# marcinmiklitz/pywindow

Measured on AMD Instinct MI355X. Metric: trajectory frames/sec full_analysis (pore+windows), CC3 1k-frame, higher is better.
Workload: dtype f64

## Files before the change

pywindow_amd/csrc/pw_kernels.hip:

```cpp
#include <hip/hip_runtime.h>
#include <atomic>
#include <stdio.h>
#include <stdlib.h>
#include <string.h>
#include <time.h>

#include <algorithm>
#include <mutex>
#include <new>

#include "../../include/pywindow_amd.h"
#include "pw_host.hpp"
#include <vector>
#include "pw_unit.hpp"
#include "pw_launch.hpp"

using namespace pw;

extern "C" int pw_hostpath_run(const pw_batch_in* in, unsigned stages, pw_unit_out* out, const pw_params* prm, int p_cap,
                               int threads, pw_unit_debug* dbg, pw_extra_window* xw, unsigned xw_cap, unsigned* xw_count);
extern "C" int pw_hostpath_default_threads(void);
extern "C" void pw_hostpath_math(int which, const double* x, const double* y, long n, double* out);
extern "C" size_t pw_internal_big_block_bytes(int nmax, int p_cap);
extern "C" int pw_internal_big_launch(void* stream, int grid, long n_units, const long* atom_offset, const double* xyz,
                                      const double* vdw, const double* mass, unsigned stages, int nmax, const PwWsArgs* wsa,
                                      unsigned char* blocks, size_t block_bytes, unsigned long long* counter, pw_unit_out* out,
                                      const pw_params* prm, const unsigned* rsq_tab, int vstride);

namespace {

thread_local char g_err[512] = "";
void set_err(const char* what, hipError_t e) {
    snprintf(g_err, sizeof(g_err), "%s: %s", what, hipGetErrorString(e));
}
#define HIP_TRY(call)                         \
    do {                                      \
        hipError_t e_ = (call);               \
        if (e_ != hipSuccess) {               \
            set_err(#call, e_);               \
            return PW_E_HIP;                  \
        }                                     \
    } while (0)

#define PW_ON_DEVICE(dev)                     \
    DeviceScope dev_scope_;                   \
    HIP_TRY(dev_scope_.enter(dev))

constexpr int PW_SETS = 4;

constexpr size_t PW_KERNEL_STATIC_LDS = 1024;

constexpr unsigned MASK_ANY = 0xffffffffu;
constexpr unsigned MASK_CHAINS = PW_STAGE_BASIC | PW_STAGE_OPT | PW_STAGE_MERGE;
constexpr unsigned MASK_WINDOWS = PW_STAGE_WINDOWS | PW_STAGE_REUSE_OPT | PW_STAGE_MERGE | PW_STAGE_COM_ONLY;
constexpr unsigned MASK_WINDOWS_AVG = MASK_WINDOWS | PW_STAGE_AVG;

__global__ void __launch_bounds__(256) pw_nb_build_kernel(unsigned* __restrict__ off, unsigned short* __restrict__ idx,
                                                          double* __restrict__ bound, double* __restrict__ unit) {
    __shared__ double ux[PW_NB_PMAX], uy[PW_NB_PMAX], uz[PW_NB_PMAX];
    const int P = PW_NB_PMAX - (int)blockIdx.x;
    Sphere sp;
    sp.init(1.0, P);
    for (int k = threadIdx.x; k < P; k += blockDim.x) sp.point(k, &ux[k], &uy[k], &uz[k]);
    __syncthreads();
    const unsigned first = nb_dense_offset(P);
    if (threadIdx.x == 0) off[P] = first;
    if (unit)
        for (int k = threadIdx.x; k < P; k += blockDim.x) {
            double* q = unit + 3 * ((size_t)first + k);
            q[0] = ux[k]; q[1] = uy[k]; q[2] = uz[k];
        }
    for (int k = threadIdx.x; k < P; k += blockDim.x)
        nb_build_point(P, k, ux, uy, uz, idx + (size_t)(first + k) * PW_NB_K, bound + first + k);
}

__device__ inline bool wait_for_unit(const unsigned long long* ready, long u, int* error_flag, long long limit) {
    if (!ready) return true;
    long long t0 = wall_clock64();
    unsigned long long seen = ~0ull;
    for (;;) {
        const unsigned long long have = __hip_atomic_load(ready, __ATOMIC_RELAXED, __HIP_MEMORY_SCOPE_SYSTEM);
        if ((long)have > u && !(have >> 63)) break;
        __builtin_amdgcn_s_sleep(16);
        if (have != seen) { seen = have; t0 = wall_clock64(); }
        if ((have >> 63) || wall_clock64() - t0 > limit) {
            if (error_flag) atomicExch(error_flag, (have >> 63) ? 3 : 2);
            return false;
        }
    }
    __builtin_amdgcn_fence(__ATOMIC_ACQUIRE, "");
    asm volatile("s_waitcnt vmcnt(0)" ::: "memory");
    return true;
}
template <int NW, unsigned MASK>
__global__ void __launch_bounds__(NW * 64, 2)
pw_analyse_kernel(long n_units, const long* __restrict__ atom_offset, const double* __restrict__ xyz,
                  const double* __restrict__ vdw, const double* __restrict__ mass, unsigned stages,
                  int nmax, int nrot, int nlb, int nframes, int lean, PwWsArgs wsa, unsigned long long* counter,
                  pw_unit_out* __restrict__ out, int role, UnitQueue* queue, int* __restrict__ slots,
                  pw_params prm_in, const unsigned* __restrict__ rsq_tab, int vstride,
                  const unsigned long long* __restrict__ ready, const unsigned char* __restrict__ tmpl) {
    extern __shared__ __attribute__((aligned(16))) unsigned char lds[];
    __shared__ long s_unit;
    __shared__ UnitShared s_sh;
    __shared__ pw_params s_prm;
    static_assert(sizeof(UnitShared) + sizeof(pw_params) + 16 <= PW_KERNEL_STATIC_LDS, "static LDS of the analysis kernels");
    using T = DeviceTeam<NW>;
    if (role == PW_ROLE_PRODUCER) {
        __builtin_amdgcn_s_setprio(3);
        if (threadIdx.x == 0) atomicAdd(&queue->started, 1);
    }
    TeamWorkspace* ws = (TeamWorkspace*)wsa.ws + blockIdx.x;
#ifdef PW_PROFILE
    if (threadIdx.x < 32) pw_prof_lds[threadIdx.x] = 0;
#ifdef PW_BARRIER_PROF
    if (threadIdx.x < 8) pw_bar_acc[threadIdx.x] = 0;
#endif
#endif
    if (threadIdx.x == 0) {
        s_sh.carve(lds, nmax, nrot, nlb, nframes, lean, wsa.p_cap);
        s_prm = prm_in;
        bind_workspace(ws, wsa, blockIdx.x, rsq_tab, team_slab_bytes(wsa.p_cap), team_adj_words(wsa.p_cap));
    }
    __syncthreads();
    constexpr bool STATE_IN_LDS = MASK == MASK_CHAINS;
    UnitShared sh_stack;
    if (!STATE_IN_LDS) sh_stack.carve(lds, nmax, nrot, nlb, nframes, lean, wsa.p_cap);
    UnitShared& sh = STATE_IN_LDS ? (UnitShared&)s_sh : sh_stack;
    const pw_params& prm = STATE_IN_LDS ? (const pw_params&)s_prm : prm_in;
    for (;;) {
        if (role == PW_ROLE_CONSUMER) {
            if (threadIdx.x == 0) {
                long pos = (long)atomicAdd(&queue->head, 1ull);
                long u = -1;
                if (pos < n_units) {
                    long long t0 = wall_clock64();
#ifdef PW_PROFILE
                    const long long t_begin = t0;
#endif
                    unsigned long long seen = ~0ull;
                    int spins = 0;
                    for (;;) {
                        int v = __hip_atomic_load(&slots[pos], __ATOMIC_RELAXED, __HIP_MEMORY_SCOPE_AGENT);
                        if (v >= 0) {
                            u = v;
#ifdef PW_PROFILE
                            atomicAdd(&pw_prof_lds[1], (unsigned long long)(wall_clock64() - t_begin));
#endif
                            break;
                        }
                        __builtin_amdgcn_s_sleep(32);
                        if (__hip_atomic_load(&queue->error, __ATOMIC_RELAXED, __HIP_MEMORY_SCOPE_AGENT) != 0) break;
                        if ((++spins & 15) == 0) {
                            const unsigned long long pub = __hip_atomic_load(&queue->tail, __ATOMIC_RELAXED, __HIP_MEMORY_SCOPE_AGENT);
                            if (pub != seen) { seen = pub; t0 = wall_clock64(); }
                        }
                        if (wall_clock64() - t0 > wsa.wait_ticks) {
                            atomicExch(&queue->error, 1);
                            break;
                        }
                    }
                    __builtin_amdgcn_fence(__ATOMIC_ACQUIRE, "agent");
                    asm volatile("s_waitcnt vmcnt(0)" ::: "memory");
                }
                s_unit = u;
            }
        } else {
            if (threadIdx.x == 0) {
                long u = (long)atomicAdd(counter, 1ull);
                if (u < n_units && !wait_for_unit(ready, u, &queue->error, wsa.stream_wait_ticks)) u = n_units;
                s_unit = u < n_units ? u : -1;
            }
        }
        __syncthreads();
        long u = s_unit;
        __syncthreads();
        if (u < 0) break;
        long a0 = atom_offset[u];
        int n = (int)(atom_offset[u + 1] - a0);
        const long v0 = a0 * vstride;
        if (threadIdx.x == 0) ws->unit = u;
        analyse_unit<T>(sh, ws, n, xyz + 3 * a0, vdw + v0, mass + v0, stages & MASK, out + u, prm, vstride == 0 ? tmpl : nullptr);
        if (role == PW_ROLE_PRODUCER) {
            if (threadIdx.x == 0) {
                asm volatile("s_waitcnt vmcnt(0)" ::: "memory");
                __builtin_amdgcn_fence(__ATOMIC_RELEASE, "agent");
                asm volatile("s_waitcnt vmcnt(0)" ::: "memory");
                long pos = (long)atomicAdd(&queue->tail, 1ull);
                __hip_atomic_store(&slots[pos], (int)u, __ATOMIC_RELAXED, __HIP_MEMORY_SCOPE_AGENT);
            }
        }
    }
#ifdef PW_PROFILE
    __syncthreads();
    if (threadIdx.x < 32 && pw_prof_lds[threadIdx.x]) atomicAdd(&ws->prof[threadIdx.x], pw_prof_lds[threadIdx.x]);
#endif
}

__global__ void pw_gate_kernel(UnitQueue* queue, int expected, unsigned long long* timeouts, long long limit) {
    if (threadIdx.x != 0) return;
    long long t0 = wall_clock64();
    int seen = -1;
    for (;;) {
        const int started = __hip_atomic_load(&queue->started, __ATOMIC_RELAXED, __HIP_MEMORY_SCOPE_AGENT);
        if (started >= expected) break;
        __builtin_amdgcn_s_sleep(16);
        if (started != seen) { seen = started; t0 = wall_clock64(); }
        if (wall_clock64() - t0 > limit) {
            atomicAdd(timeouts, 1ull << 32);
            if (started == 0) atomicCAS(&queue->error, 0, 4);
            break;
        }
    }
}

__global__ void pw_tail_gate_kernel(const UnitQueue* prev, unsigned long long need, unsigned long long* timeouts) {
    if (threadIdx.x != 0) return;
    long long t0 = wall_clock64();
    while (__hip_atomic_load(&prev->tail, __ATOMIC_RELAXED, __HIP_MEMORY_SCOPE_AGENT) < need) {
        __builtin_amdgcn_s_sleep(32);
        if (wall_clock64() - t0 > 2000000ll) { atomicAdd(timeouts, 1ull); break; }
    }
}

__global__ void pw_head_gate_kernel(const UnitQueue* prev, unsigned long long need, unsigned long long* timeouts) {
    if (threadIdx.x != 0) return;
    long long t0 = wall_clock64();
    while (__hip_atomic_load(&prev->head, __ATOMIC_RELAXED, __HIP_MEMORY_SCOPE_AGENT) < need) {
        __builtin_amdgcn_s_sleep(32);
        if (wall_clock64() - t0 > 2000000ll) { atomicAdd(timeouts, 1ull << 16); break; }
    }
}

__global__ void pw_probe_kernel(int* started, int expected, int* together) {
    if (threadIdx.x != 0) return;
    atomicAdd(started, 1);
    long long t0 = wall_clock64();
    while (__hip_atomic_load(started, __ATOMIC_RELAXED, __HIP_MEMORY_SCOPE_AGENT) < expected) {
        __builtin_amdgcn_s_sleep(16);
        if (wall_clock64() - t0 > 1000000ll) return;
    }
    atomicAdd(together, 1);
}

template <int NW>
__global__ void __launch_bounds__(NW * 64) pw_dbscan_kernel(const double* __restrict__ pts, int n, double eps,
                                                            int lds_bytes, TeamWorkspace* ws, int p_cap,
                                                            unsigned long long* adj_base, const int* __restrict__ ident,
                                                            int* __restrict__ labels, int* __restrict__ n_clusters) {
    using T = DeviceTeam<NW>;
    extern __shared__ __attribute__((aligned(16))) unsigned char lds[];
    __shared__ unsigned long long bits[3][PW_DBSCAN_MAX / 64];
    if (threadIdx.x == 0) { ws->adj = adj_base; ws->p_cap = p_cap; }
    __syncthreads();
    ScratchArena arena;
    arena.cur = (unsigned char*)lds;
    arena.left = (size_t)lds_bytes;
    int* lab = (int*)arena.take((size_t)n * 4);
    if (!lab) lab = labels;
    auto PT = [n](int k, int c) { return c * n + k; };
    int k = team_dbscan<T>((PW_LDS unsigned long long*)bits[0], (PW_LDS unsigned long long*)bits[1],
                           (PW_LDS unsigned long long*)bits[2], arena, ws, pts, PT, ident, n, eps, lab);
    if (lab != labels)
        for (int i = threadIdx.x; i < n; i += NW * 64) labels[i] = lab[i];
    if (threadIdx.x == 0) *n_clusters = k;
}

template <int NW>
__global__ void __launch_bounds__(NW * 64) pw_pairwise_sum_kernel(const double* __restrict__ a, long n,
                                                                   double* __restrict__ scratch, int use_global,
                                                                   double* __restrict__ out) {
    using T = DeviceTeam<NW>;
    __shared__ int s_tab[324];
    __shared__ double s_acc[8 * 160];
    __shared__ double s_leaf[256];
    __shared__ double s_slot;
    int* tab = use_global ? (int*)(scratch + 8 * 160 + 256) : (int*)s_tab;
    double* acc = use_global ? scratch : (double*)s_acc;
// ... 1724 lines not shown
        if (d_p) (void)hipFree(d_p);
        if (d_i) (void)hipFree(d_i);
        if (d_l) (void)hipFree(d_l);
        if (d_ws) (void)hipFree(d_ws);
        if (d_adj) (void)hipFree(d_adj);
    };
#define DB_TRY(call)                                   \
    do {                                               \
        hipError_t e_ = (call);                        \
        if (e_ != hipSuccess) {                        \
            set_err(#call, e_);                        \
            cleanup();                                 \
            return PW_E_HIP;                           \
        }                                              \
    } while (0)
    std::vector<double> soa((size_t)3 * n);
    std::vector<int> ident((size_t)n);
    for (int64_t i = 0; i < n; ++i) {
        for (int k = 0; k < 3; ++k) soa[(size_t)k * n + i] = points[3 * i + k];
        ident[i] = (int)i;
    }
    DB_TRY(hipMalloc((void**)&d_p, sizeof(double) * 3 * n));
    DB_TRY(hipMalloc((void**)&d_i, sizeof(int) * n));
    DB_TRY(hipMalloc((void**)&d_l, sizeof(int) * (n + 1)));
    DB_TRY(hipMalloc((void**)&d_ws, sizeof(TeamWorkspace)));
    const int p_cap = round_p_cap((long)n);
    DB_TRY(hipMalloc((void**)&d_adj, sizeof(unsigned long long) * team_adj_words(p_cap)));
    DB_TRY(hipMemcpyAsync(d_p, soa.data(), sizeof(double) * 3 * n, hipMemcpyHostToDevice, c->stream));
    DB_TRY(hipMemcpyAsync(d_i, ident.data(), sizeof(int) * n, hipMemcpyHostToDevice, c->stream));
    const int lds_bytes = (mode & 2) ? 0 : 96 * 1024;
    if (mode & 1) {
        DB_TRY(hipFuncSetAttribute((const void*)pw_dbscan_kernel<1>, hipFuncAttributeMaxDynamicSharedMemorySize, 96 * 1024));
        hipLaunchKernelGGL(pw_dbscan_kernel<1>, dim3(1), dim3(64), lds_bytes, c->stream, d_p, (int)n, eps, lds_bytes, d_ws, p_cap,
                           d_adj, d_i, d_l, d_l + n);
    } else {
        DB_TRY(hipFuncSetAttribute((const void*)pw_dbscan_kernel<4>, hipFuncAttributeMaxDynamicSharedMemorySize, 96 * 1024));
        hipLaunchKernelGGL(pw_dbscan_kernel<4>, dim3(1), dim3(256), lds_bytes, c->stream, d_p, (int)n, eps, lds_bytes, d_ws, p_cap,
                           d_adj, d_i, d_l, d_l + n);
    }
    DB_TRY(hipGetLastError());
    DB_TRY(hipMemcpyAsync(labels, d_l, sizeof(int) * n, hipMemcpyDeviceToHost, c->stream));
    DB_TRY(hipMemcpyAsync(n_clusters, d_l + n, sizeof(int), hipMemcpyDeviceToHost, c->stream));
    DB_TRY(hipStreamSynchronize(c->stream));
#undef DB_TRY
    cleanup();
    return PW_OK;
}

int pw_pairwise_sum(pw_context* c, const double* values, int64_t n, int mode, double* sum) {
    if (!c || !sum || n < 0 || n > 0x7fffffff || (n > 0 && !values)) return PW_E_BAD_ARG;
    PW_LOCK_CONTEXT(c);
    PW_HOST_UNSUPPORTED(c, "pw_pairwise_sum");
    PW_ON_DEVICE(c->device);
    double *d_a = nullptr, *d_s = nullptr;
    auto cleanup = [&]() {
        if (d_a) (void)hipFree(d_a);
        if (d_s) (void)hipFree(d_s);
    };
#define PS_TRY(call)                                   \
    do {                                               \
        hipError_t e_ = (call);                        \
        if (e_ != hipSuccess) {                        \
            set_err(#call, e_);                        \
            cleanup();                                 \
            return PW_E_HIP;                           \
        }                                              \
    } while (0)
    const size_t scratch_doubles = 8 * 160 + 256 + 324 / 2 + 2;
    PS_TRY(hipMalloc((void**)&d_a, sizeof(double) * (size_t)(n > 0 ? n : 1)));
    PS_TRY(hipMalloc((void**)&d_s, sizeof(double) * scratch_doubles));
    if (n > 0) PS_TRY(hipMemcpyAsync(d_a, values, sizeof(double) * (size_t)n, hipMemcpyHostToDevice, c->stream));
    if (mode & 1)
        hipLaunchKernelGGL(pw_pairwise_sum_kernel<1>, dim3(1), dim3(64), 0, c->stream, d_a, (long)n, d_s + 1, (mode >> 1) & 1, d_s);
    else
        hipLaunchKernelGGL(pw_pairwise_sum_kernel<4>, dim3(1), dim3(256), 0, c->stream, d_a, (long)n, d_s + 1, (mode >> 1) & 1, d_s);
    PS_TRY(hipGetLastError());
    PS_TRY(hipMemcpyAsync(sum, d_s, sizeof(double), hipMemcpyDeviceToHost, c->stream));
    PS_TRY(hipStreamSynchronize(c->stream));
#undef PS_TRY
    cleanup();
    return PW_OK;
}

int pw_debug_stage_ticks(pw_context* c, unsigned long long* out32) {
#ifdef PW_PROFILE
    if (!c || !out32 || !c->ws) return PW_E_BAD_ARG;
    HIP_TRY(hipStreamSynchronize(c->stream));
    for (int i = 0; i < 32; ++i) out32[i] = 0;
    for (int b = 0; b < c->ws_blocks; ++b) {
        unsigned long long tmp[32];
        HIP_TRY(hipMemcpy(tmp, c->ws[b].prof, sizeof(tmp), hipMemcpyDeviceToHost));
        for (int i = 0; i < 32; ++i) out32[i] += tmp[i];
        HIP_TRY(hipMemset(c->ws[b].prof, 0, sizeof(tmp)));
    }
    return PW_OK;
#else
    (void)c; (void)out32;
    return PW_E_BAD_ARG;
#endif
}

}
```

pywindow_amd/csrc/pw_lbfgsb.hpp:

```cpp
#pragma once
#include "pw_blas.hpp"
#include "pw_team.hpp"

#if defined(PW_PROFILE) && defined(__HIP_DEVICE_COMPILE__)
#define LB_T0(var) long long var = wall_clock64()
#define LB_T1(slot, var) do { if (prof && T::lane() == 0) atomicAdd(&prof[slot], (unsigned long long)(wall_clock64() - var)); } while (0)
#else
#define LB_T0(var) do {} while (0)
#define LB_T1(slot, var) do {} while (0)
#endif
#if defined(PW_PROFILE) && defined(PW_LB_FINE) && defined(__HIP_DEVICE_COMPILE__)
#define LB_F0(var) long long var = clock64()
#define LB_F1(slot, var) do { if (prof && T::lane() == 0) atomicAdd(&prof[slot], (unsigned long long)(clock64() - var)); } while (0)
#define LB_M0(var) long long var = clock64()
#define LB_M1(slot, var) do { if (m->prof_fine && T::lane() == 0) atomicAdd(&m->prof_fine[slot], (unsigned long long)(clock64() - var)); } while (0)
#else
#define LB_F0(var) do {} while (0)
#define LB_F1(slot, var) do {} while (0)
#define LB_M0(var) do {} while (0)
#define LB_M1(slot, var) do {} while (0)
#endif

namespace pw {

enum LbTask : int {
    LB_START = 0,
    LB_NEW_X = 1,
    LB_FG = 3,
    LB_CONVERGENCE = 4,
    LB_STOP = 5,
    LB_WARNING = 6,
    LB_ERROR = 7,
    LB_ABNORMAL = 8,
};
enum LbMsg : int {
    LBM_NONE = 0,
    LBM_FG_START = 301,
    LBM_FG_LNSRCH = 302,
    LBM_CONV_PGTOL = 401,
    LBM_CONV_FTOL = 402,
};

constexpr int LB_M = 10;

struct LsState {
    double ginit, gtest, gx, gy, finit, fx, fy, stx, sty, stmin, stmax, width, width1;
    int brackt, stage;
};

template <int N>
struct LbMem {
    static constexpr int M = LB_M;
    static constexpr int M2 = 2 * LB_M;
    double l[N], u[N];
    double x[N], g[N];
    double ws[M * N], wy[M * N];
    double sy[M * M], ss[M * M], wt[M * M];
    double wn[M2 * M2], wn1d[M2];
    double z[N], r[N], d[N], t[N], xp[N];
    double wa[8 * M];
    double acc[2 * M];
    double dsy[M], rsy[M], sqy[M], rsq[M], rwt[M], rwn[M2];
    double iwn[M];
    double tri[64];
    int pair[64];
    double le[N], ue[N];
    LsState ls;
#if defined(PW_PROFILE) && defined(PW_LB_FINE)
    unsigned long long* prof_fine;
#endif
    int cand[32];
    int nbd[N];
    int index[N], iwhere[N], indx2[N];
};

template <class T>
PW_NOINLINE PW_HD inline void lb_trsv_un_wave(int n, const double* a, int lda, double* x) {
    PW_ASSUME_LDS(a);
    PW_ASSUME_LDS(x);
    const int lane = T::lane();
    double xk = lane < n ? x[lane] : 0.0;
    for (int i = n - 1; i >= 0; --i) {
        const double* ci = a + (long)i * lda;
        double xi = T::bcast_u(xk, i) / ci[i];
        if (lane == i) xk = xi;
        if (lane < i) xk = pw_fma(-xi, ci[lane], xk);
    }
    T::wave_sync();
    if (lane < n) x[lane] = xk;
    T::wave_sync();
}
template <class T>
PW_NOINLINE PW_HD inline void lb_trsv_ut_wave(int n, const double* a, int lda, double* x) {
    PW_ASSUME_LDS(a);
    PW_ASSUME_LDS(x);
    const int lane = T::lane();
    const double* ci = a + (long)(lane < n ? lane : 0) * lda;
    double xk = lane < n ? x[lane] : 0.0;
    double ak = 0.0;
    for (int s = 0; s < n; ++s) {
        double xs = T::bcast_u(xk, s);
        if (s > 0) xs = xs - T::bcast_u(ak, s);
        xs = xs / a[s + (long)s * lda];
        if (lane == s) xk = xs;
        if (lane > s && lane < n) {
            if (lane >= 16 && s < 16) {
                if (s == 15) {
                    double sl[4];
                    for (int l = 0; l < 4; ++l) {
                        double a0 = ci[l] * T::bcast_u(xk, l);
                        double a1 = ci[4 + l] * T::bcast_u(xk, 4 + l);
                        double a2 = ci[8 + l] * T::bcast_u(xk, 8 + l);
                        double a3 = ci[12 + l] * T::bcast_u(xk, 12 + l);
                        sl[l] = ((a0 + a1) + a2) + a3;
                    }
                    ak = (sl[0] + sl[2]) + (sl[1] + sl[3]);
                }
            } else {
                ak = pw_fma(xs, ci[s], ak);
            }
        }
    }
    T::wave_sync();
    if (lane < n) x[lane] = xk;
    T::wave_sync();
}


#if defined(__HIP_DEVICE_COMPILE__)
typedef DeviceTeam<1> LbWave;
__device__ inline int lb_uniform(int v) { return __builtin_amdgcn_readfirstlane(v); }
template <class P>
__device__ inline P* lb_uniform(P* p) {
    union { P* p; int i[2]; } a;
    a.p = p;
    a.i[0] = __builtin_amdgcn_readfirstlane(a.i[0]);
    a.i[1] = __builtin_amdgcn_readfirstlane(a.i[1]);
    return a.p;
}
template <class T, int NMAX, bool SPEC>
__device__ inline __attribute__((always_inline)) double lb_solve_ut_reg(int n, const double* a, int lda, const double* rdiag,
                                                                       double xk, double* tnum) {
    PW_ASSUME_LDS(a);
    PW_ASSUME_LDS(rdiag);
    const int lane = T::lane();
    const bool act = lane < n;
    const int li = act ? lane : 0;
    const double* ci = a + li * lda;
    double c[NMAX];
#pragma unroll
    for (int k = 0; k < NMAX; ++k) c[k] = ci[k];
    int dli = li * (lda + 1);
    asm volatile("" : "+v"(dli));
    double dg = a[dli], rd = rdiag[li];
// ... 2151 lines not shown
```

pywindow_amd/csrc/pw_unit.hpp:

```cpp
#pragma once
#include "../../include/pywindow_amd.h"
#include "pw_lbfgsb.hpp"
#include "pw_math.hpp"
#include "pw_team.hpp"
#include <string.h>

#if defined(PW_PROFILE) && defined(__HIPCC__)
__shared__ unsigned long long pw_prof_lds[32];
#define PW_PROF_BASE(ws) ((unsigned long long*)pw_prof_lds)
#endif
#if defined(PW_PROFILE) && defined(__HIP_DEVICE_COMPILE__)
#define PW_T0(var) long long var = wall_clock64()
#if defined(PW_ZPROF) && defined(PW_LB_FINE)
#define PW_T1(ws, slot, var) do { (void)var; } while (0)
#elif defined(PW_BARRIER_PROF)
#define PW_T1(ws, slot, var) do { (void)var; if (T::lane() == 0) { unsigned long long w_ = 0; \
        for (int k_ = 0; k_ < T::NWAVES; ++k_) w_ += atomicExch(&pw_bar_acc[k_], 0ull); \
        atomicAdd(&pw_prof_lds[slot], w_); } } while (0)
#else
#define PW_T1(ws, slot, var) do { if (T::lane() == 0) atomicAdd(&pw_prof_lds[slot], (unsigned long long)(wall_clock64() - var)); } while (0)
#endif
#else
#define PW_T0(var) do {} while (0)
#define PW_T1(ws, slot, var) do {} while (0)
#endif

namespace pw {

constexpr double GOLDEN_ANGLE = 2.399963229728653;
constexpr double FOUR_PI = 12.566370614359172;
constexpr double FOUR_THIRDS_PI = 4.1887902047863905;
constexpr double TWO_PI = 6.283185307179586;
constexpr double ONE_PI = 3.141592653589793;

constexpr int PW_KCLS = 8;
constexpr double PW_PATH_POINTS_MAX = 1048576.0;
struct ClassInfo {
    int k;
    int off[PW_KCLS + 1];
    double vdw[PW_KCLS];
};
struct Frame {
    ldouble *x, *y, *z, *xx;
    const ldouble* vdw;
    const lint* perm;
    const PW_LDS ClassInfo* cls;
};

struct TeamWorkspace {
    double* knn;
    double* pts;
    double* vals;
    int* surv_k;
    int* labels;
    unsigned char* flag;
    unsigned long long* adj;
    double* xw;
    int* xw_ok;
    int p_cap;
    const unsigned* nb_off;
    const unsigned short* nb_idx;
    const double* nb_unit;
    const double* nb_bound;
    pw_extra_window* xwin;
    unsigned* xwin_count;
    unsigned xwin_cap;
    double leaf[256];
    double acc8[8 * 160];
    int leaf_tab[324];
    unsigned long long prof[32];
    const unsigned* rsq;
    pw_unit_debug* dbg_base;
    long unit;
};
PW_HD inline size_t team_slab_bytes(int p_cap) { return (size_t)p_cap * 192; }
PW_HD inline size_t team_adj_words(int p_cap) { return (size_t)p_cap * (size_t)(p_cap / 64); }
PW_HD inline int round_p_cap(long p) {
    if (p < PW_P_MAX) p = PW_P_MAX;
    return (int)((p + 127) & ~127l);
}
PW_HD inline int params_p_cap(double adjust_windows, double adjust_average) {
    double a = adjust_windows > adjust_average ? adjust_windows : adjust_average;
    if (!(a > 0.0)) a = 1.0;
    double want = 2100.0 * a;
    if (want > 4.0e6) want = 4.0e6;
    return round_p_cap((long)want + 1);
}
PW_HD inline void bind_team_slab(TeamWorkspace* ws, unsigned char* slab, int p_cap) {
    const size_t p = (size_t)p_cap;
    double* d = (double*)slab;
    ws->knn = d; d += 10 * p;
    ws->pts = d; d += 3 * p;
// ... 252 lines not shown
        const double r = C.vdw[g];
#pragma unroll
        for (int p = 0; p < NP; ++p) {
            const double m2p = m2[p] + pp[p];
            double d = pw_sqrt(m2p > 0.0 ? m2p : 0.0);
            best[p] = __builtin_fmin(best[p], d - r);
        }
    }
#pragma unroll
    for (int p = 0; p < NP; ++p) out[p] = best[p];
}

template <class T>
PW_HD inline double wave_gap(const Frame& F, int n, double px, double py, double pz, int* arg) {
    double pp = sq3(px, py, pz);
    double best = PW_INF;
    int bi = 0x7fffffff;
    for (int i = T::lane(); i < n; i += T::WSIZE) {
        double v = gap_atom(F, i, px, py, pz, pp);
        int oi = F.perm[i];
        if (v < best || (v == best && oi < bi)) { best = v; bi = oi; }
    }
    T::wave_argmin(best, bi);
    if (arg) *arg = bi;
    return best;
}

template <class T>
PW_HD inline double wave_gap_value(const Frame& F, int n, double px, double py, double pz) {
    double pp = sq3(px, py, pz);
    double best = PW_INF;
    for (int i = T::lane(); i < n; i += T::WSIZE) best = __builtin_fmin(best, gap_atom(F, i, px, py, pz, pp));
    return T::wave_min(best);
}

template <class T>
PW_HD inline void wave_gap4(const Frame& F, int n, const double* px, const double* py,
                            const double* pz, double* out) {
    if (T::WSIZE == 64) {
        int g = T::lane() >> 4, l = T::lane() & 15;
        double qx = g == 0 ? px[0] : (g == 1 ? px[1] : (g == 2 ? px[2] : px[3]));
        double qy = g == 0 ? py[0] : (g == 1 ? py[1] : (g == 2 ? py[2] : py[3]));
        double qz = g == 0 ? pz[0] : (g == 1 ? pz[1] : (g == 2 ? pz[2] : pz[3]));
        double pp = sq3(qx, qy, qz);
        double best = PW_INF;
        const auto& C = *F.cls;
        const int kk = T::uniform_i(C.k);
        if (kk > 0) {
            for (int c = 0; c < kk; ++c) {
                const int lo = T::uniform_i(C.off[c]), hi = T::uniform_i(C.off[c + 1]);
                double m2 = PW_INF;
                int base = lo;
                for (; base + 16 < hi; base += 32) {
                    int i0 = base + l, i1 = base + 16 + l;
                    i1 = i1 < hi ? i1 : hi - 1;
                    const double x0 = F.x[i0], y0 = F.y[i0], z0 = F.z[i0], s0 = F.xx[i0];
                    const double x1 = F.x[i1], y1 = F.y[i1], z1 = F.z[i1], s1 = F.xx[i1];
                    const double g0 = pw_fma(z0, qz, pw_fma(x0, qx, y0 * qy));
                    const double g1 = pw_fma(z1, qz, pw_fma(x1, qx, y1 * qy));
                    m2 = __builtin_fmin(m2, pw_m2add(g0, s0));
                    m2 = __builtin_fmin(m2, pw_m2add(g1, s1));
                }
                if (base < hi) {
                    int i0 = base + l;
                    i0 = i0 < hi ? i0 : hi - 1;
                    const double gg = pw_fma(F.z[i0], qz, pw_fma(F.x[i0], qx, F.y[i0] * qy));
                    m2 = __builtin_fmin(m2, pw_m2add(gg, F.xx[i0]));
                }
                m2 = m2 + pp;
                const double d = pw_sqrt(m2 > 0.0 ? m2 : 0.0);
                best = __builtin_fmin(best, d - C.vdw[c]);
            }
        } else {
#pragma unroll 4
            for (int i = l; i < n; i += 16) best = __builtin_fmin(best, gap_atom(F, i, qx, qy, qz, pp));
        }
        T::row_min4(best, out);
    } else {
        for (int q = 0; q < 4; ++q) out[q] = wave_gap<T>(F, n, px[q], py[q], pz[q], nullptr);
    }
}

#if defined(__HIP_DEVICE_COMPILE__)
struct NearList4 { int c0, c1, total; };
struct NearList1 { int mine, total; };
template <class T>
PW_NOINLINE __device__ inline NearList4 near_rebuild4(Frame F, int n, PW_LDS int* cand, double px, double py, double pz,
                                                      double slack) {
    const int lane = T::lane();
    const double pp = sq3(px, py, pz);
    double best = PW_INF;
    for (int i = lane; i < n; i += 64) best = __builtin_fmin(best, gap_atom(F, i, px, py, pz, pp));
    best = T::wave_min(best);
    const double lim = best + slack;
    int total = 0;
    for (int i0 = 0; i0 < n; i0 += 64) {
        const int i = i0 + lane;
        const bool in = i < n && gap_atom(F, i < n ? i : 0, px, py, pz, pp) <= lim;
        const unsigned long long m = T::ballot(in);
        const int at = total + (int)__builtin_popcountll(m & ((1ull << lane) - 1ull));
        if (in && at < 32) cand[at] = i;
        total += (int)__builtin_popcountll(m);
    }
    T::wave_sync();
    NearList4 r;
    r.c0 = r.c1 = -1;
    if (!(pp < 1.0e9)) total = 1 << 20;
    r.total = total;
    const int l = lane & 15;
    if (total <= 32) {
        if (l < total) r.c0 = cand[l];
        if (l + 16 < total) r.c1 = cand[l + 16];
    }
    T::wave_sync();
    return r;
}
template <class T>
PW_NOINLINE __device__ inline NearList1 near_rebuild1(Frame F, int n, double px, double py, double pz, double slack) {
    const int lane = T::lane();
    const double pp = sq3(px, py, pz);
    double best = PW_INF;
    for (int i = lane; i < n; i += 64) best = __builtin_fmin(best, gap_atom(F, i, px, py, pz, pp));
    best = T::wave_min(best);
    const double lim = best + slack;
    NearList1 r;
    r.mine = -1;
    int total = 0;
    for (int i0 = 0; i0 < n; i0 += 64) {
        const int i = i0 + lane;
        const bool in = i < n && gap_atom(F, i < n ? i : 0, px, py, pz, pp) <= lim;
        const unsigned long long m = T::ballot(in);
        const int cnt = (int)__builtin_popcountll(m);
        const int want = lane - total;
        if (want >= 0 && want < cnt) {
            unsigned long long mm = m;
            for (int k = 0; k < want; ++k) mm &= mm - 1ull;
            r.mine = i0 + (int)__builtin_ctzll(mm);
        }
        total += cnt;
    }
    if (!(pp < 1.0e9)) total = 1 << 20;
    r.total = total;
    return r;
}
template <class T>
struct NearGap4 {
    static constexpr double DELTA = 0.3, MARGIN = 1e-6;
    double rx, ry, rz;
    int c0, c1;
    int state;

    __device__ void init() { rx = ry = rz = 0.0; c0 = c1 = -1; state = 0; }

    __device__ void rebuild(const Frame& F, int n, PW_LDS int* cand, double px, double py, double pz) {
        const NearList4 r = near_rebuild4<T>(F, n, cand, px, py, pz, 2.0 * DELTA + MARGIN);
        rx = px; ry = py; rz = pz;
        c0 = r.c0; c1 = r.c1;
        state = r.total <= 32 ? 1 : 2;
    }

    __device__ void eval(const Frame& F, int n, PW_LDS int* cand, const double* px, const double* py, const double* pz,
                         double* out) {
        const int g = T::lane() >> 4;
        const double qx = g == 0 ? px[0] : (g == 1 ? px[1] : (g == 2 ? px[2] : px[3]));
        const double qy = g == 0 ? py[0] : (g == 1 ? py[1] : (g == 2 ? py[2] : py[3]));
        const double qz = g == 0 ? pz[0] : (g == 1 ? pz[1] : (g == 2 ? pz[2] : pz[3]));
        const bool near = pw_abs(qx - rx) + pw_abs(qy - ry) + pw_abs(qz - rz) <= DELTA;
        if (state == 0 || !T::wave_all(near)) rebuild(F, n, cand, px[0], py[0], pz[0]);
        const bool near2 = pw_abs(qx - rx) + pw_abs(qy - ry) + pw_abs(qz - rz) <= DELTA;
        if (state != 1 || !T::wave_all(near2)) {
            wave_gap4<T>(F, n, px, py, pz, out);
            return;
        }
        const double pp = sq3(qx, qy, qz);
        const int i0 = c0 < 0 ? 0 : c0, i1 = c1 < 0 ? 0 : c1;
        const double x0 = F.x[i0], y0 = F.y[i0], z0 = F.z[i0], s0 = F.xx[i0], r0 = F.vdw[i0];
        const double x1 = F.x[i1], y1 = F.y[i1], z1 = F.z[i1], s1 = F.xx[i1], r1 = F.vdw[i1];
        const double g0 = pw_fma(z0, qz, pw_fma(x0, qx, y0 * qy));
        const double g1 = pw_fma(z1, qz, pw_fma(x1, qx, y1 * qy));
        const double d0 = pw_m2add(g0, s0) + pp, d1 = pw_m2add(g1, s1) + pp;
        const double v0 = pw_sqrt(d0 > 0.0 ? d0 : 0.0) - r0, v1 = pw_sqrt(d1 > 0.0 ? d1 : 0.0) - r1;
        double best = c0 < 0 ? PW_INF : v0;
        best = c1 < 0 ? best : __builtin_fmin(best, v1);
        T::row_min4(best, out);
    }
};
template <class T>
struct NearGap1 {
    static constexpr double DELTA = 0.3, MARGIN = 1e-6;
    double rx, ry, rz;
    int c;
    int state;
    double ax, ay, az, aq, ar;

    __device__ void init() { rx = ry = rz = 0.0; c = -1; state = 0; ax = ay = az = aq = ar = 0.0; }

    __device__ void rebuild(const Frame& F, int n, PW_LDS int* cand, double px, double py, double pz) {
        (void)cand;
        const NearList1 r = near_rebuild1<T>(F, n, px, py, pz, 2.0 * DELTA + MARGIN);
        rx = px; ry = py; rz = pz;
        c = r.total <= 64 ? r.mine : -1;
        state = r.total <= 64 ? 1 : 2;
        const int i = c < 0 ? 0 : c;
        ax = F.x[i]; ay = F.y[i]; az = F.z[i]; aq = F.xx[i]; ar = F.vdw[i];
    }

    __device__ double eval(const Frame& F, int n, PW_LDS int* cand, double px, double py, double pz) {
        const bool near = pw_abs(px - rx) + pw_abs(py - ry) + pw_abs(pz - rz) <= DELTA;
        if (state == 0 || !T::wave_all(near)) rebuild(F, n, cand, px, py, pz);
        if (state != 1) return wave_gap_value<T>(F, n, px, py, pz);
        const double g = pw_fma(az, pz, pw_fma(ax, px, ay * py));
        const double d2 = pw_m2add(g, aq) + sq3(px, py, pz);
        const double v = pw_sqrt(d2 > 0.0 ? d2 : 0.0) - ar;
        return T::wave_min(c < 0 ? PW_INF : v);
    }
};
#endif

PW_HD inline double np_leaf_sum(const double* a, int n) {
    if (n < 8) {
        double r = 0.0;
        for (int i = 0; i < n; ++i) r = r + a[i];
        return r;
    }
    double r0 = a[0], r1 = a[1], r2 = a[2], r3 = a[3], r4 = a[4], r5 = a[5], r6 = a[6], r7 = a[7];
    int i = 8;
    int lim = n - (n % 8);
    for (; i < lim; i += 8) {
        r0 += a[i]; r1 += a[i + 1]; r2 += a[i + 2]; r3 += a[i + 3];
        r4 += a[i + 4]; r5 += a[i + 5]; r6 += a[i + 6]; r7 += a[i + 7];
    }
    double res = ((r0 + r1) + (r2 + r3)) + ((r4 + r5) + (r6 + r7));
    for (; i < n; ++i) res = res + a[i];
    return res;
}
struct NpSeg { int off, len, stage; };
PW_HD inline int np_leaves(int off, int n, int* loff, int* llen) {
    NpSeg st[24];
    int top = 0, nl = 0;
    st[top++] = NpSeg{off, n, 0};
    while (top) {
        NpSeg c = st[--top];
        if (c.len <= 128) {
            loff[nl] = c.off; llen[nl] = c.len; ++nl;
        } else {
            int n2 = c.len / 2;
            n2 -= n2 % 8;
            st[top++] = NpSeg{c.off + n2, c.len - n2, 0};
            st[top++] = NpSeg{c.off, n2, 0};
        }
    }
    return nl;
}
PW_HD inline double np_combine(int n, const double* leafsum) {
    NpSeg st[24];
    double vals[24];
    int top = 0, vtop = 0, li = 0;
    st[top++] = NpSeg{0, n, 0};
    while (top) {
        NpSeg& c = st[top - 1];
        if (c.len <= 128) {
            vals[vtop++] = leafsum[li++];
            --top;
        } else if (c.stage == 0) {
            int n2 = c.len / 2;
            n2 -= n2 % 8;
            c.stage = 1;
            st[top++] = NpSeg{c.off, n2, 0};
        } else if (c.stage == 1) {
            int n2 = c.len / 2;
            n2 -= n2 % 8;
            c.stage = 2;
            int o = c.off, l = c.len;
            st[top++] = NpSeg{o + n2, l - n2, 0};
        } else {
            double r = vals[--vtop];
            double l = vals[--vtop];
            vals[vtop++] = l + r;
            --top;
        }
    }
    return vals[0];
}
PW_HD inline double np_sum_small(const double* a, int n) {
    NpSeg st[24];
    double vals[24];
    int top = 0, vtop = 0;
    st[top++] = NpSeg{0, n, 0};
    while (top) {
        NpSeg& c = st[top - 1];
        if (c.len <= 128) {
            vals[vtop++] = np_leaf_sum(a + c.off, c.len);
            --top;
// ... 1612 lines not shown
    auto sort3 = [&]() {
        if (f0s > f1s) swap01();
        if (f1s > f2s) { swap12(); if (f0s > f1s) swap01(); }
    };
    sort3();
    int iterations = 1;
    while (fcalls < maxfun && iterations < maxiter) {
        double dx1 = pw_abs(x1s - x0s), dx2 = pw_abs(x2s - x0s);
        double dy1 = pw_abs(y1s - y0s), dy2 = pw_abs(y2s - y0s);
        double mx = pw_max(pw_max(dx1, dy1), pw_max(dx2, dy2));
        double mf = pw_max(pw_abs(f0s - f1s), pw_abs(f0s - f2s));
        if (mx <= xatol && mf <= fatol) break;
        double bx = (x0s + x1s) / 2.0, by = (y0s + y1s) / 2.0;
        double xr = 2.0 * bx - x2s, yr = 2.0 * by - y2s;
        bool over = false;
        auto guarded = [&](double x, double y, double* f) {
            if (fcalls >= maxfun) { over = true; return false; }
            *f = fun(x, y);
            return true;
        };
        double fxr;
        if (guarded(xr, yr, &fxr)) {
            bool doshrink = false;
            if (fxr < f0s) {
                double xe = 3.0 * bx - 2.0 * x2s, ye = 3.0 * by - 2.0 * y2s;
                double fxe;
                if (guarded(xe, ye, &fxe)) {
                    if (fxe < fxr) { x2s = xe; y2s = ye; f2s = fxe; }
                    else { x2s = xr; y2s = yr; f2s = fxr; }
                }
            } else if (fxr < f1s) {
                x2s = xr; y2s = yr; f2s = fxr;
            } else if (fxr < f2s) {
                double xc = 1.5 * bx - 0.5 * x2s, yc = 1.5 * by - 0.5 * y2s;
                double fxc;
                if (guarded(xc, yc, &fxc)) {
                    if (fxc <= fxr) { x2s = xc; y2s = yc; f2s = fxc; }
                    else doshrink = true;
                }
            } else {
                double xcc = 0.5 * bx + 0.5 * x2s, ycc = 0.5 * by + 0.5 * y2s;
                double fxcc;
                if (guarded(xcc, ycc, &fxcc)) {
                    if (fxcc < f2s) { x2s = xcc; y2s = ycc; f2s = fxcc; }
                    else doshrink = true;
                }
            }
            if (doshrink && !over) {
                x1s = x0s + 0.5 * (x1s - x0s);
                y1s = y0s + 0.5 * (y1s - y0s);
                double f;
                if (guarded(x1s, y1s, &f)) f1s = f;
                if (!over) {
                    x2s = x0s + 0.5 * (x2s - x0s);
                    y2s = y0s + 0.5 * (y2s - y0s);
                    if (guarded(x2s, y2s, &f)) f2s = f;
                }
            }
            if (!over) iterations += 1;
        }
        sort3();
    }
    *xo = x0s;
    *yo = y0s;
    *n_eval += fcalls;
}

template <class T>
struct NeckObjective {
    const Frame& R;
    int n;
    double xo, yo, lo, up;
    PW_LDS int* cand;
    bool have_last;
    double lz, lf, lg;
    int nfev;
#if defined(__HIP_DEVICE_COMPILE__)
    NearGap4<T> near_gap;
#endif
    PW_HD NeckObjective(const Frame& R_, int n_, double xo_, double yo_, double lo_, double up_, PW_LDS int* cand_)
        : R(R_), n(n_), xo(xo_), yo(yo_), lo(lo_), up(up_), cand(cand_), have_last(false), lz(0.0), lf(0.0), lg(0.0), nfev(0) {
#if defined(__HIP_DEVICE_COMPILE__)
        near_gap.init();
#endif
    }
    PW_HD __attribute__((always_inline)) void operator()(const double* xq, double& fo, double* go) {
        const double zc = xq[0];
        if (!(have_last && zc == lz)) {
            double h = fd_step(zc, lo, up);
            double z1 = zc + h;
            double dz = z1 - zc;
            double zx[4] = {xo, xo, xo, xo}, zy[4] = {yo, yo, yo, yo}, zz[4] = {zc, z1, zc, z1}, gv[4];
#if defined(__HIP_DEVICE_COMPILE__)
            if (T::WSIZE == 64) near_gap.eval(R, n, cand, zx, zy, zz, gv);
            else
#endif
            wave_gap4<T>(R, n, zx, zy, zz, gv);
            double f0 = gv[0] * 2.0;
            double f1 = gv[1] * 2.0;
            nfev += 2;
            lf = f0;
            lg = (f1 - f0) / dz;
            lz = zc;
            have_last = true;
        }
        fo = lf;
        go[0] = lg;
    }
};

#if defined(__HIP_DEVICE_COMPILE__)
template <class T>
PW_NOINLINE __device__ inline bool wave_brute_bounded(Frame R, int n, PW_LDS double* scratch, int cap, double zopt,
                                                      double gstart, double gstep, int* gidx_out) {
    constexpr double TAU = 0.7;
    const PW_LDS ClassInfo* C = R.cls;
    const int kk = T::uniform_i(C->k);
    cap = T::uniform_i(cap);
    n = T::uniform_i(n);
    if (kk == 0 || cap < 16 || n > 256) return false;
    PW_LDS double *sx = scratch, *sy = scratch + cap, *sz = scratch + 2 * cap, *sq = scratch + 3 * cap;
    const int lane = T::lane();
    const double cx = 9.5 * gstep + gstart, cy = cx;
    const double ppc = sq3(cx, cy, zopt);
    double ax[4], ay[4], az[4], aq[4], ag[4];
    double b = PW_INF;
#pragma unroll
    for (int t = 0; t < 4; ++t) {
        const int i = lane + 64 * t;
        const int ic = i < n ? i : 0;
        ax[t] = R.x[ic]; ay[t] = R.y[ic]; az[t] = R.z[ic]; aq[t] = R.xx[ic];
        const double gg = pw_fma(az[t], zopt, pw_fma(ax[t], cx, ay[t] * cy));
        const double d2 = pw_m2add(gg, aq[t]) + ppc;
        ag[t] = i < n ? pw_sqrt(d2 > 0.0 ? d2 : 0.0) - R.vdw[ic] : PW_INF;
        b = __builtin_fmin(b, ag[t]);
    }
    const double lim = T::wave_min(b) + TAU;
    if (!(lim < PW_INF)) return false;
    int coff[PW_KCLS + 1];
#pragma unroll
    for (int g = 0; g <= PW_KCLS; ++g) coff[g] = 0;
    int total = 0;
#pragma unroll
    for (int t = 0; t < 4; ++t) {
        if (64 * t >= n) continue;
        const bool in = ag[t] <= lim;
        const unsigned long long mk = T::ballot(in);
        const int at = total + (int)__builtin_popcountll(mk & ((1ull << lane) - 1ull));
        if (in && at < cap) { sx[at] = ax[t]; sy[at] = ay[t]; sz[at] = az[t]; sq[at] = aq[t]; }
#pragma unroll
        for (int g = 0; g <= PW_KCLS; ++g) {
            const int first = g < kk ? T::uniform_i(C->off[g]) : n;
            const int below = first - 64 * t;
            const unsigned long long lt = below >= 64 ? ~0ull : (below <= 0 ? 0ull : ((1ull << below) - 1ull));
            coff[g] += (int)__builtin_popcountll(mk & lt);
        }
        total += (int)__builtin_popcountll(mk);
    }
    if (total > cap || total == 0) return false;
    T::wave_sync();
    double qx[7], qy[7], pp[7], ub[7];
#pragma unroll
    for (int p = 0; p < 7; ++p) {
        int q = lane + 64 * p;
        if (q >= 400) q = lane;
        qx[p] = (double)(q / 20) * gstep + gstart;
// ... 1277 lines not shown
```

Before: 978,600.

## Cache a wide near-atom list to speed near-list rebuilds in L-BFGS-B gap evaluation

Adds a second-level 'wide' candidate list (up to 128 atom indices within a larger slack) stored in LDS after cand[], built during full rebuilds. Later rebuilds within a wider radius scan only the wide list instead of all atoms. For n<=256 the full scan also caches per-lane gap values in registers so they are not recomputed in the second pass. It also adds optional profiling counters, which are compiled out by default. The cost is extra LDS per workspace and more register pressure in the rebuild routines.

```diff
diff --git a/pywindow_amd/csrc/pw_kernels.hip b/pywindow_amd/csrc/pw_kernels.hip
--- a/pywindow_amd/csrc/pw_kernels.hip
+++ b/pywindow_amd/csrc/pw_kernels.hip
@@ -92,6 +92,9 @@
     asm volatile("s_waitcnt vmcnt(0)" ::: "memory");
     return true;
 }
+#if defined(PW_PROFILE) && defined(PW_LB_FINE)
+__device__ unsigned long long pw_near_counts[48];
+#endif
 template <int NW, unsigned MASK>
 __global__ void __launch_bounds__(NW * 64, 2)
 pw_analyse_kernel(long n_units, const long* __restrict__ atom_offset, const double* __restrict__ xyz,
@@ -113,6 +116,9 @@
     TeamWorkspace* ws = (TeamWorkspace*)wsa.ws + blockIdx.x;
 #ifdef PW_PROFILE
     if (threadIdx.x < 32) pw_prof_lds[threadIdx.x] = 0;
+#ifdef PW_LB_FINE
+    if (threadIdx.x < 48) pw_near_lds[threadIdx.x] = 0;
+#endif
 #ifdef PW_BARRIER_PROF
     if (threadIdx.x < 8) pw_bar_acc[threadIdx.x] = 0;
 #endif
@@ -194,6 +200,9 @@
 #ifdef PW_PROFILE
     __syncthreads();
     if (threadIdx.x < 32 && pw_prof_lds[threadIdx.x]) atomicAdd(&ws->prof[threadIdx.x], pw_prof_lds[threadIdx.x]);
+#ifdef PW_LB_FINE
+    if (threadIdx.x < 48 && pw_near_lds[threadIdx.x]) atomicAdd(&pw_near_counts[threadIdx.x], pw_near_lds[threadIdx.x]);
+#endif
 #endif
 }
 
@@ -2084,6 +2093,21 @@
     return PW_OK;
 }
 
+int pw_debug_near_counts(pw_context* c, unsigned long long* out48) {
+#if defined(PW_PROFILE) && defined(PW_LB_FINE)
+    if (!c || !out48) return PW_E_BAD_ARG;
+    HIP_TRY(hipStreamSynchronize(c->stream));
+    HIP_TRY(hipDeviceSynchronize());
+    HIP_TRY(hipMemcpyFromSymbol(out48, HIP_SYMBOL(pw_near_counts), 48 * sizeof(unsigned long long)));
+    unsigned long long zero[48] = {0};
+    HIP_TRY(hipMemcpyToSymbol(HIP_SYMBOL(pw_near_counts), zero, sizeof(zero)));
+    return PW_OK;
+#else
+    (void)c; (void)out48;
+    return PW_E_BAD_ARG;
+#endif
+}
+
 int pw_debug_stage_ticks(pw_context* c, unsigned long long* out32) {
 #ifdef PW_PROFILE
     if (!c || !out32 || !c->ws) return PW_E_BAD_ARG;
diff --git a/pywindow_amd/csrc/pw_lbfgsb.hpp b/pywindow_amd/csrc/pw_lbfgsb.hpp
--- a/pywindow_amd/csrc/pw_lbfgsb.hpp
+++ b/pywindow_amd/csrc/pw_lbfgsb.hpp
@@ -46,6 +46,13 @@
 struct LsState {
     double ginit, gtest, gx, gy, finit, fx, fy, stx, sty, stmin, stmax, width, width1;
     int brackt, stage;
+};
+
+constexpr int LB_NEAR_WIDE = 128;
+struct NearWideList {
+    double rx, ry, rz;
+    int n, pad;
+    unsigned char at[LB_NEAR_WIDE];
 };
 
 template <int N>
@@ -70,6 +77,7 @@
     unsigned long long* prof_fine;
 #endif
     int cand[32];
+    NearWideList wide;
     int nbd[N];
     int index[N], iwhere[N], indx2[N];
 };
diff --git a/pywindow_amd/csrc/pw_unit.hpp b/pywindow_amd/csrc/pw_unit.hpp
--- a/pywindow_amd/csrc/pw_unit.hpp
+++ b/pywindow_amd/csrc/pw_unit.hpp
@@ -8,6 +8,9 @@
 #if defined(PW_PROFILE) && defined(__HIPCC__)
 __shared__ unsigned long long pw_prof_lds[32];
 #define PW_PROF_BASE(ws) ((unsigned long long*)pw_prof_lds)
+#if defined(PW_LB_FINE)
+__shared__ unsigned long long pw_near_lds[48];
+#endif
 #endif
 #if defined(PW_PROFILE) && defined(__HIP_DEVICE_COMPILE__)
 #define PW_T0(var) long long var = wall_clock64()
@@ -426,31 +429,96 @@
 }
 
 #if defined(__HIP_DEVICE_COMPILE__)
+constexpr double NEAR_DELTA = 0.3, NEAR_MARGIN = 1e-6, NEAR_DELTA_WIDE = 1.2;
+static_assert(offsetof(LbMem<3>, wide) == offsetof(LbMem<3>, cand) + 128 && offsetof(LbMem<1>, wide) == offsetof(LbMem<1>, cand) + 128 &&
+              offsetof(LbMem<3>, wide) % 8 == 0 && offsetof(LbMem<1>, wide) % 8 == 0, "the wide list follows cand[32]");
+constexpr double NEAR_SLACK = 2.0 * NEAR_DELTA + NEAR_MARGIN, NEAR_SLACK_WIDE = 2.0 * NEAR_DELTA_WIDE + 2.0 * NEAR_MARGIN;
+#if defined(PW_PROFILE) && defined(PW_LB_FINE)
+#define PW_NEAR_CNT(who, slot, val) do { if (T::lane() == 0) atomicAdd(&pw_near_lds[16 * (who) + (slot)], (unsigned long long)(val)); } while (0)
+#define PW_NEAR_LEN(who, total, cap) PW_NEAR_CNT(who, (total) > (cap) ? 13 : ((total) > 48 ? 12 : 6 + ((total) - 1) / 8), 1)
+struct NearList4 { int c0, c1, total, via_wide; };
+#else
+#define PW_NEAR_CNT(who, slot, val) do {} while (0)
+#define PW_NEAR_LEN(who, total, cap) do {} while (0)
 struct NearList4 { int c0, c1, total; };
+#endif
 struct NearList1 { int mine, total; };
 template <class T>
 PW_NOINLINE __device__ inline NearList4 near_rebuild4(Frame F, int n, PW_LDS int* cand, double px, double py, double pz,
-                                                      double slack) {
+                                                      int fresh) {
     const int lane = T::lane();
     const double pp = sq3(px, py, pz);
-    double best = PW_INF;
-    for (int i = lane; i < n; i += 64) best = __builtin_fmin(best, gap_atom(F, i, px, py, pz, pp));
-    best = T::wave_min(best);
-    const double lim = best + slack;
+    auto* W = (PW_LDS NearWideList*)(cand + 32);
     int total = 0;
-    for (int i0 = 0; i0 < n; i0 += 64) {
-        const int i = i0 + lane;
-        const bool in = i < n && gap_atom(F, i < n ? i : 0, px, py, pz, pp) <= lim;
+    n = T::uniform_i(n);
+    const int wn = fresh ? 0 : T::uniform_i(W->n);
+    bool use_wide = false;
+    if (wn > 0) use_wide = T::wave_all(pw_abs(px - W->rx) + pw_abs(py - W->ry) + pw_abs(pz - W->rz) <= NEAR_DELTA_WIDE - NEAR_DELTA);
+    auto append = [&](bool in, int i) {
         const unsigned long long m = T::ballot(in);
         const int at = total + (int)__builtin_popcountll(m & ((1ull << lane) - 1ull));
         if (in && at < 32) cand[at] = i;
         total += (int)__builtin_popcountll(m);
+    };
+    if (use_wide) {
+        const int a0 = lane < wn ? (int)W->at[lane] : -1;
+        const int a1 = lane + 64 < wn ? (int)W->at[lane + 64] : -1;
+        const double g0 = a0 < 0 ? PW_INF : gap_atom(F, a0 < 0 ? 0 : a0, px, py, pz, pp);
+        double g1 = PW_INF;
+        if (wn > 64) g1 = a1 < 0 ? PW_INF : gap_atom(F, a1 < 0 ? 0 : a1, px, py, pz, pp);
+        const double lim = T::wave_min(__builtin_fmin(g0, g1)) + NEAR_SLACK;
+        append(a0 >= 0 && g0 <= lim, a0);
+        if (wn > 64) append(a1 >= 0 && g1 <= lim, a1);
+    } else if (n <= 256) {
+        double g[4];
+        double best = PW_INF;
+#pragma unroll
+        for (int t = 0; t < 4; ++t) {
+            g[t] = PW_INF;
+            if (64 * t < n) {
+                const int i = 64 * t + lane;
+                if (i < n) g[t] = gap_atom(F, i, px, py, pz, pp);
+                best = __builtin_fmin(best, g[t]);
+            }
+        }
+        best = T::wave_min(best);
+        const double lim = best + NEAR_SLACK, wlim = best + NEAR_SLACK_WIDE;
+        int wtotal = 0;
+#pragma unroll
+        for (int t = 0; t < 4; ++t) {
+            if (64 * t < n) {
+                const int i = 64 * t + lane;
+                append(i < n && g[t] <= lim, i);
+                const bool win = i < n && g[t] <= wlim;
+                const unsigned long long m = T::ballot(win);
+                const int at = wtotal + (int)__builtin_popcountll(m & ((1ull << lane) - 1ull));
+                if (win && at < LB_NEAR_WIDE) W->at[at] = (unsigned char)i;
+                wtotal += (int)__builtin_popcountll(m);
+            }
+        }
+        if (lane == 0) {
+            W->rx = px; W->ry = py; W->rz = pz;
+            W->n = (wtotal <= LB_NEAR_WIDE && pp < 1.0e9) ? wtotal : 0;
+        }
+    } else {
+        double best = PW_INF;
+        for (int i = lane; i < n; i += 64) best = __builtin_fmin(best, gap_atom(F, i, px, py, pz, pp));
+        best = T::wave_min(best);
+        const double lim = best + NEAR_SLACK;
+        for (int i0 = 0; i0 < n; i0 += 64) {
+            const int i = i0 + lane;
+            append(i < n && gap_atom(F, i < n ? i : 0, px, py, pz, pp) <= lim, i);
+        }
+        if (lane == 0) W->n = 0;
     }
     T::wave_sync();
     NearList4 r;
     r.c0 = r.c1 = -1;
     if (!(pp < 1.0e9)) total = 1 << 20;
     r.total = total;
+#if defined(PW_PROFILE) && defined(PW_LB_FINE)
+    r.via_wide = use_wide;
+#endif
     const int l = lane & 15;
     if (total <= 32) {
         if (l < total) r.c0 = cand[l];
@@ -460,19 +528,14 @@
     return r;
 }
 template <class T>
-PW_NOINLINE __device__ inline NearList1 near_rebuild1(Frame F, int n, double px, double py, double pz, double slack) {
+PW_NOINLINE __device__ inline NearList1 near_rebuild1(Frame F, int n, double px, double py, double pz) {
     const int lane = T::lane();
     const double pp = sq3(px, py, pz);
-    double best = PW_INF;
-    for (int i = lane; i < n; i += 64) best = __builtin_fmin(best, gap_atom(F, i, px, py, pz, pp));
-    best = T::wave_min(best);
-    const double lim = best + slack;
     NearList1 r;
     r.mine = -1;
     int total = 0;
-    for (int i0 = 0; i0 < n; i0 += 64) {
-        const int i = i0 + lane;
-        const bool in = i < n && gap_atom(F, i < n ? i : 0, px, py, pz, pp) <= lim;
+    n = T::uniform_i(n);
+    auto append = [&](bool in, int i0) {
         const unsigned long long m = T::ballot(in);
         const int cnt = (int)__builtin_popcountll(m);
         const int want = lane - total;
@@ -482,6 +545,31 @@
             r.mine = i0 + (int)__builtin_ctzll(mm);
         }
         total += cnt;
+    };
+    if (n <= 256) {
+        double g[4];
+        double best = PW_INF;
+#pragma unroll
+        for (int t = 0; t < 4; ++t) {
+            g[t] = PW_INF;
+            if (64 * t < n) {
+                const int i = 64 * t + lane;
+                if (i < n) g[t] = gap_atom(F, i, px, py, pz, pp);
+                best = __builtin_fmin(best, g[t]);
+            }
+        }
+        const double lim = T::wave_min(best) + NEAR_SLACK;
+#pragma unroll
+        for (int t = 0; t < 4; ++t)
+            if (64 * t < n) append(64 * t + lane < n && g[t] <= lim, 64 * t);
+    } else {
+        double best = PW_INF;
+        for (int i = lane; i < n; i += 64) best = __builtin_fmin(best, gap_atom(F, i, px, py, pz, pp));
+        const double lim = T::wave_min(best) + NEAR_SLACK;
+        for (int i0 = 0; i0 < n; i0 += 64) {
+            const int i = i0 + lane;
+            append(i < n && gap_atom(F, i < n ? i : 0, px, py, pz, pp) <= lim, i0);
+        }
     }
     if (!(pp < 1.0e9)) total = 1 << 20;
     r.total = total;
@@ -489,15 +577,28 @@
 }
 template <class T>
 struct NearGap4 {
-    static constexpr double DELTA = 0.3, MARGIN = 1e-6;
+    static constexpr double DELTA = NEAR_DELTA;
     double rx, ry, rz;
     int c0, c1;
     int state;
-
+#if defined(PW_PROFILE) && defined(PW_LB_FINE)
+    int who;
+    __device__ void init() { rx = ry = rz = 0.0; c0 = c1 = -1; state = 0; who = 0; }
+#else
     __device__ void init() { rx = ry = rz = 0.0; c0 = c1 = -1; state = 0; }
+#endif
 
     __device__ void rebuild(const Frame& F, int n, PW_LDS int* cand, double px, double py, double pz) {
-        const NearList4 r = near_rebuild4<T>(F, n, cand, px, py, pz, 2.0 * DELTA + MARGIN);
+#if defined(PW_PROFILE) && defined(PW_LB_FINE)
+        const long long t0 = clock64();
+#endif
+        const NearList4 r = near_rebuild4<T>(F, n, cand, px, py, pz, state == 0);
+#if defined(PW_PROFILE) && defined(PW_LB_FINE)
+        PW_NEAR_CNT(who, 4, clock64() - t0);
+        PW_NEAR_CNT(who, r.via_wide ? 2 : 1, 1);
+        PW_NEAR_CNT(who, 5, r.total <= 32 ? r.total : 0);
+        PW_NEAR_LEN(who, r.total, 32);
+#endif
         rx = px; ry = py; rz = pz;
         c0 = r.c0; c1 = r.c1;
         state = r.total <= 32 ? 1 : 2;
@@ -510,9 +611,11 @@
         const double qy = g == 0 ? py[0] : (g == 1 ? py[1] : (g == 2 ? py[2] : py[3]));
         const double qz = g == 0 ? pz[0] : (g == 1 ? pz[1] : (g == 2 ? pz[2] : pz[3]));
         const bool near = pw_abs(qx - rx) + pw_abs(qy - ry) + pw_abs(qz - rz) <= DELTA;
+        PW_NEAR_CNT(who, 0, 1);
         if (state == 0 || !T::wave_all(near)) rebuild(F, n, cand, px[0], py[0], pz[0]);
         const bool near2 = pw_abs(qx - rx) + pw_abs(qy - ry) + pw_abs(qz - rz) <= DELTA;
         if (state != 1 || !T::wave_all(near2)) {
+            PW_NEAR_CNT(who, 3, 1);
             wave_gap4<T>(F, n, px, py, pz, out);
             return;
         }
@@ -531,7 +634,7 @@
 };
 template <class T>
 struct NearGap1 {
-    static constexpr double DELTA = 0.3, MARGIN = 1e-6;
+    static constexpr double DELTA = NEAR_DELTA;
     double rx, ry, rz;
     int c;
     int state;
@@ -541,7 +644,16 @@
 
     __device__ void rebuild(const Frame& F, int n, PW_LDS int* cand, double px, double py, double pz) {
         (void)cand;
-        const NearList1 r = near_rebuild1<T>(F, n, px, py, pz, 2.0 * DELTA + MARGIN);
+#if defined(PW_PROFILE) && defined(PW_LB_FINE)
+        const long long t0 = clock64();
+#endif
+        const NearList1 r = near_rebuild1<T>(F, n, px, py, pz);
+#if defined(PW_PROFILE) && defined(PW_LB_FINE)
+        PW_NEAR_CNT(2, 4, clock64() - t0);
+        PW_NEAR_CNT(2, 1, 1);
+        PW_NEAR_CNT(2, 5, r.total <= 64 ? r.total : 0);
+        PW_NEAR_LEN(2, r.total, 64);
+#endif
         rx = px; ry = py; rz = pz;
         c = r.total <= 64 ? r.mine : -1;
         state = r.total <= 64 ? 1 : 2;
@@ -551,8 +663,12 @@
 
     __device__ double eval(const Frame& F, int n, PW_LDS int* cand, double px, double py, double pz) {
         const bool near = pw_abs(px - rx) + pw_abs(py - ry) + pw_abs(pz - rz) <= DELTA;
+        PW_NEAR_CNT(2, 0, 1);
         if (state == 0 || !T::wave_all(near)) rebuild(F, n, cand, px, py, pz);
-        if (state != 1) return wave_gap_value<T>(F, n, px, py, pz);
+        if (state != 1) {
+            PW_NEAR_CNT(2, 3, 1);
+            return wave_gap_value<T>(F, n, px, py, pz);
+        }
         const double g = pw_fma(az, pz, pw_fma(ax, px, ay * py));
         const double d2 = pw_m2add(g, aq) + sq3(px, py, pz);
         const double v = pw_sqrt(d2 > 0.0 ? d2 : 0.0) - ar;
@@ -2331,6 +2447,9 @@
         : R(R_), n(n_), xo(xo_), yo(yo_), lo(lo_), up(up_), cand(cand_), have_last(false), lz(0.0), lf(0.0), lg(0.0), nfev(0) {
 #if defined(__HIP_DEVICE_COMPILE__)
         near_gap.init();
+#if defined(PW_PROFILE) && defined(PW_LB_FINE)
+        near_gap.who = 1;
+#endif
 #endif
     }
     PW_HD __attribute__((always_inline)) void operator()(const double* xq, double& fo, double* go) {
```

New measurement: 981,100 (median of 6 runs). Within noise of the previous version (+0.3%).
